# jammm/first_raytracer

Hardware: AMD Instinct MI355X
Metric: Mrays/sec + RMSE vs CPU ref, CornellBox 1080p 512spp, 1/2/4/8 MI355X (higher is better)
Workload: dtype f32

## Files before the change

first_raytracer_amd/__init__.py:

```python
import ctypes
import os

import numpy as np

HERE = os.path.dirname(os.path.abspath(__file__))
LIB_PATH = os.environ.get("FRT_LIB_PATH") or os.path.join(HERE, "libfrt.so")

FRT_WORLD_BVH, FRT_WORLD_LIST = 0, 1
FRT_MAT_LAMBERTIAN, FRT_MAT_DIFFUSE_LIGHT = 0, 1
FRT_PRIM_SPHERE = 1 << 30
ABI_VERSION = 9
FRT_MAT_LAMBERTIAN, FRT_MAT_DIFFUSE_LIGHT, FRT_MAT_MODIFIED_PHONG, FRT_MAT_METAL, FRT_MAT_DIELECTRIC = 0, 1, 2, 3, 4
FRT_MAT_ROUGH_CONDUCTOR = 5
FRT_DIST_GGX, FRT_DIST_BECKMANN = 0, 1
FRT_TEX_CONSTANT, FRT_TEX_CHECKER, FRT_TEX_IMAGE = 0, 1, 2
FRT_IMAGE_SRGB8, FRT_IMAGE_F32 = 0, 1
FRT_FLAG_NO_LDS_SCENE = 1
FRT_FLAG_WAVES5 = 2
FRT_FLAG_WAVES6 = 4
FRT_FLAG_WAVES4 = 8
FRT_FLAG_BVH2 = 16
FRT_FLAG_NO_OCT = 256
FRT_FLAG_FP64 = 512
FRT_FLAG_FP32 = 1024
# ... 96 lines not shown

    @classmethod
    def make(cls, nx, ny, spp, seed=0, max_depth=33, tile_size=32, shard_index=0, shard_count=1,
             samples_per_item=0, flags=0, integrator=0, sample_offset=0):
        return cls(nx=nx, ny=ny, spp=spp, seed=seed, max_depth=max_depth, integrator=integrator, tile_size=tile_size,
                   shard_index=shard_index, shard_count=shard_count, samples_per_item=samples_per_item, flags=flags,
                   mlt_chains=0, mlt_bootstrap=0, sample_offset=sample_offset)

    @classmethod
    def pssmlt(cls, nx, ny, mutations_per_pixel, chains, seed=0, bootstrap=10000, shard_index=0, shard_count=1,
               flags=0):
        return cls(nx=nx, ny=ny, spp=mutations_per_pixel, seed=seed, max_depth=10, integrator=FRT_INTEGRATOR_PSSMLT,
                   tile_size=32, shard_index=shard_index, shard_count=shard_count, samples_per_item=0, flags=flags,
                   mlt_chains=chains, mlt_bootstrap=bootstrap)


class Stats(ctypes.Structure):
    _fields_ = [(n, ctypes.c_uint64) for n in ("camera_rays", "extension_rays", "shadow_rays", "samples",
                                               "pixels", "work_items")] + [
        ("kernel_ms", ctypes.c_double), ("total_ms", ctypes.c_double)] + [
        (n, ctypes.c_uint32) for n in ("scene_in_lds", "waves_cap", "stack_entries", "bvh_depth")] + [
        ("scene_bytes", ctypes.c_uint64), ("fp64", ctypes.c_uint32), ("reserved", ctypes.c_uint32)]

    @property
    def rays(self):
        return self.camera_rays + self.extension_rays + self.shadow_rays

    def as_dict(self):
        d = {n: getattr(self, n) for n, _ in self._fields_}
        d["rays"] = self.rays
        return d


class HostSceneInfo(ctypes.Structure):
    _fields_ = [(n, ctypes.c_int32) for n in ("n_tris", "n_spheres", "n_materials", "n_lights", "n_nodes",
                                              "world_kind", "n_list", "bvh_depth")] + [
        ("load_ms", ctypes.c_double), ("build_ms", ctypes.c_double)]


_lib = None

EXPORTS = ("frt_get_abi_version", "frt_create", "frt_destroy", "frt_last_error", "frt_set_precision", "frt_upload_scene",
           "frt_shard_slot_count", "frt_shard_slots", "frt_render", "frt_render_multi", "frt_render_device", "frt_trace_device",
           "frt_mlt_chain_state",
           "frt_scene_create", "frt_scene_new", "frt_scene_add_obj", "frt_scene_add_sphere", "frt_scene_set_camera",
           "frt_scene_set_env", "frt_scene_add_image", "frt_scene_finish", "frt_scene_build_bvh_gpu",
           "frt_scene_build_bvh_sah", "frt_scene_build_bvh_gpu_algo",
           "frt_scene_view_get", "frt_scene_info", "frt_scene_destroy", "frt_write_tessellated_obj",
           "frt_write_pfm", "frt_film_accumulate", "frt_tonemap_u8", "frt_write_image", "frt_selftest_path_host",
           "frt_selftest_mlt_paths_host",
           "frt_set_env_image", "frt_scene_set_env_image", "frt_scene_env_image", "frt_read_hdr",
           "frt_selftest_path_host_env")


def lib():
    global _lib
    if _lib is not None:
        return _lib
    if not os.path.exists(LIB_PATH):
        raise FrtError(f"{LIB_PATH} is missing: build it with `python -c 'import __graft_entry__ as g; g.build()'`")
    try:
        import torch
    except ImportError:
        pass
    L = ctypes.CDLL(LIB_PATH)
    vp = ctypes.c_void_p
    L.frt_get_abi_version.restype = ctypes.c_int
    if L.frt_get_abi_version() != ABI_VERSION:
        raise FrtError(f"{LIB_PATH}: ABI version {L.frt_get_abi_version()}, binding expects {ABI_VERSION}; rebuild")
    L.frt_create.argtypes = [ctypes.c_int, ctypes.POINTER(vp)]
    L.frt_destroy.argtypes = [vp]
    L.frt_last_error.argtypes = [vp]
    L.frt_last_error.restype = ctypes.c_char_p
    L.frt_set_precision.argtypes = [vp, ctypes.c_int]
    L.frt_upload_scene.argtypes = [vp, ctypes.POINTER(SceneView)]
    L.frt_shard_slot_count.argtypes = [ctypes.POINTER(RenderParams)]
    L.frt_shard_slot_count.restype = ctypes.c_int64
    L.frt_shard_slots.argtypes = [ctypes.POINTER(RenderParams), vp]
    L.frt_render.argtypes = [vp, ctypes.POINTER(RenderParams), vp, ctypes.POINTER(Stats)]
    L.frt_render_device.argtypes = [vp, ctypes.POINTER(RenderParams), vp, vp, ctypes.POINTER(Stats)]
    L.frt_trace_device.argtypes = [vp, vp, ctypes.c_int64, vp, ctypes.c_int, vp, ctypes.POINTER(Stats)]
    L.frt_mlt_chain_state.argtypes = [vp, ctypes.c_uint64, ctypes.c_uint64, vp, vp]
    L.frt_render_multi.argtypes = [ctypes.POINTER(vp), ctypes.c_int, ctypes.POINTER(RenderParams), vp,
                                   ctypes.POINTER(Stats)]
    L.frt_scene_create.argtypes = [ctypes.c_char_p, ctypes.c_char_p, ctypes.c_double, ctypes.POINTER(vp)]
    L.frt_scene_view_get.argtypes = [vp, ctypes.POINTER(SceneView)]
    L.frt_scene_info.argtypes = [vp, ctypes.POINTER(HostSceneInfo)]
    L.frt_scene_destroy.argtypes = [vp]
    L.frt_scene_destroy.restype = None
    dp = ctypes.POINTER(ctypes.c_double)
    L.frt_scene_new.argtypes = [ctypes.POINTER(vp)]
    L.frt_scene_add_obj.argtypes = [vp, ctypes.c_char_p, dp, ctypes.POINTER(Material), ctypes.c_int]
    L.frt_scene_add_sphere.argtypes = [vp, dp, ctypes.c_double, ctypes.POINTER(Material), ctypes.c_int]
    L.frt_scene_set_camera.argtypes = [vp, dp, dp, dp, ctypes.c_double, ctypes.c_double, ctypes.c_double,
                                       ctypes.c_double]
    L.frt_scene_set_env.argtypes = [vp, dp]
    L.frt_scene_add_image.argtypes = [vp, ctypes.POINTER(Image), ctypes.POINTER(ctypes.c_int)]
    L.frt_scene_finish.argtypes = [vp, ctypes.c_int]
    L.frt_scene_build_bvh_gpu.argtypes = [vp, vp, ctypes.POINTER(ctypes.c_double)]
    L.frt_scene_build_bvh_sah.argtypes = [vp]
    L.frt_scene_build_bvh_gpu_algo.argtypes = [vp, vp, ctypes.c_int, ctypes.POINTER(ctypes.c_double)]
    L.frt_write_tessellated_obj.argtypes = [ctypes.c_char_p, ctypes.c_int, ctypes.c_char_p]
    L.frt_write_pfm.argtypes = [ctypes.c_char_p, ctypes.c_int, ctypes.c_int, vp]
    L.frt_film_accumulate.argtypes = [vp, ctypes.c_int64, vp, ctypes.c_int64, ctypes.c_int64]
    L.frt_tonemap_u8.argtypes = [vp, ctypes.c_int, ctypes.c_int, vp]
    L.frt_write_image.argtypes = [ctypes.c_char_p, ctypes.c_int, ctypes.c_int, vp, ctypes.c_int]
    L.frt_selftest_path_host.argtypes = [ctypes.POINTER(SceneView), ctypes.POINTER(RenderParams), vp,
                                         ctypes.c_int, vp, ctypes.POINTER(Stats)]
    L.frt_selftest_mlt_paths_host.argtypes = [ctypes.POINTER(SceneView), ctypes.c_int, ctypes.c_int, ctypes.c_uint32,
                                              ctypes.c_int, vp]
    L.frt_set_env_image.argtypes = [vp, ctypes.POINTER(Image)]
    L.frt_scene_set_env_image.argtypes = [vp, ctypes.c_int]
    L.frt_scene_env_image.argtypes = [vp, ctypes.POINTER(Image)]
    L.frt_read_hdr.argtypes = [ctypes.c_char_p, ctypes.POINTER(ctypes.c_int32), ctypes.POINTER(ctypes.c_int32), vp]
    L.frt_selftest_path_host_env.argtypes = [ctypes.POINTER(SceneView), ctypes.POINTER(RenderParams), vp,
                                             ctypes.c_int, ctypes.POINTER(Image), vp, ctypes.POINTER(Stats)]
    _lib = L
    return L


def _check(rc, what, ctx=None):
    if rc != 0:
        msg = ""
        if ctx is not None:
            msg = lib().frt_last_error(ctx).decode(errors="replace")
        raise FrtError(f"{what} failed: {ERRORS.get(rc, rc)} {msg}")


class HostScene:

    def __init__(self, kind, obj_path, aspect):
        self.ptr = ctypes.c_void_p()
        _check(lib().frt_scene_create(kind.encode(), obj_path.encode(), float(aspect), ctypes.byref(self.ptr)),
               f"frt_scene_create({kind})")
        self.info = HostSceneInfo()
        lib().frt_scene_info(self.ptr, ctypes.byref(self.info))
        self.env = None

    def set_env(self, rgb):
        self.env = tuple(float(x) for x in rgb)

    def set_env_image(self, index):
        _check(lib().frt_scene_set_env_image(self.ptr, -1 if index is None else int(index)), "frt_scene_set_env_image")

    def env_image(self):
        img = Image()
        rc = lib().frt_scene_env_image(self.ptr, ctypes.byref(img))
        if rc < 0:
            _check(rc, "frt_scene_env_image")
# ... 176 lines not shown
    arr = (ctypes.c_void_p * len(contexts))(*[c.ptr for c in contexts])
    st = Stats()
    _check(lib().frt_render_multi(arr, len(contexts), ctypes.byref(params), film.ctypes.data, ctypes.byref(st)),
           "frt_render_multi", contexts[0].ptr)
    return film, st


def shard_slots(params):
    n = lib().frt_shard_slot_count(ctypes.byref(params))
    if n < 0:
        raise FrtError("bad render params")
    out = np.zeros(n, np.int32)
    _check(lib().frt_shard_slots(ctypes.byref(params), out.ctypes.data), "frt_shard_slots")
    return out


def selftest_path_host(scene, params, pixels, env_image=None):
    pixels = np.ascontiguousarray(pixels, dtype=np.int32)
    out = np.zeros((len(pixels), 3), np.float32)
    st = Stats()
    view = scene.view()
    if env_image is None:
        _check(lib().frt_selftest_path_host(ctypes.byref(view), ctypes.byref(params), pixels.ctypes.data, len(pixels),
                                            out.ctypes.data, ctypes.byref(st)), "frt_selftest_path_host")
        return out, st
    a, fmt = image_array({"data": env_image})
    desc = Image(a.shape[1], a.shape[0], fmt, 0, a.ctypes.data)
    _check(lib().frt_selftest_path_host_env(ctypes.byref(view), ctypes.byref(params), pixels.ctypes.data, len(pixels),
                                            ctypes.byref(desc), out.ctypes.data, ctypes.byref(st)),
           "frt_selftest_path_host_env")
    return out, st


def selftest_mlt_paths_host(scene, nx, ny, seed, n):
    out = np.zeros((n, 6), np.float32)
    view = scene.view()
    _check(lib().frt_selftest_mlt_paths_host(ctypes.byref(view), nx, ny, seed, n, out.ctypes.data),
           "frt_selftest_mlt_paths_host")
    return out


def read_hdr(path):
    nx, ny = ctypes.c_int32(0), ctypes.c_int32(0)
    _check(lib().frt_read_hdr(os.fsencode(path), ctypes.byref(nx), ctypes.byref(ny), None), f"frt_read_hdr({path})")
    out = np.zeros((ny.value, nx.value, 3), np.float32)
    _check(lib().frt_read_hdr(os.fsencode(path), ctypes.byref(nx), ctypes.byref(ny), out.ctypes.data),
           f"frt_read_hdr({path})")
    return out


def write_pfm(path, film):
    film = np.ascontiguousarray(film, dtype=np.float32)
    ny, nx = film.shape[0], film.shape[1]
    _check(lib().frt_write_pfm(path.encode(), nx, ny, film.ctypes.data), "frt_write_pfm")


def film_accumulate(acc, acc_spp, film, spp):
    acc = np.ascontiguousarray(acc, dtype=np.float32)
    film = np.ascontiguousarray(film, dtype=np.float32)
    _check(lib().frt_film_accumulate(acc.ctypes.data, int(acc_spp), film.ctypes.data, int(spp), film.size),
           "frt_film_accumulate")
    return acc


def tonemap_u8(film):
    film = np.ascontiguousarray(film, dtype=np.float32)
# ... 28 lines not shown
```

first_raytracer_amd/csrc/frt_flatten.hip:

```cpp
#include "frt_flatten.hpp"

#include <algorithm>
#include <cfloat>
#include <cmath>
#include <cstdlib>
#include <functional>

#include "frt_kernels.hpp"

using namespace frt;

static inline float round_down(double x)
{
    float f = (float)x;
    if ((double)f > x) f = std::nextafter(f, -INFINITY);
    return f;
}
static inline float round_up(double x)
{
    float f = (float)x;
    if ((double)f < x) f = std::nextafter(f, INFINITY);
    return f;
}

static int leaf_size_override()
{
    const char *e = std::getenv("FRT_LEAF_SIZE");
    return e ? std::min(std::max(std::atoi(e), 1), kLeafMax) : 0;
}

static void collapse_leaves(FlatScene &F, int leaf_max)
{
    const int nn = (int)(F.nodes.size() / 4);
    if (leaf_max <= 1 || nn == 0) return;
    auto child = [&](int i, int side) { return f2i(side ? F.nodes[4 * i + 3].y : F.nodes[4 * i + 3].x); };
    std::vector<int> cnt(nn, 0), first(nn, INT32_MAX);
    std::vector<char> sph(nn, 0);
    for (int i = nn - 1; i >= 0; --i)
        for (int side = 0; side < 2; ++side) {
            const int c = child(i, side);
            if (c >= 0) {
// ... 159 lines not shown
    auto srgb = [](double v) { return v <= 0.04045 ? v * (1.0 / 12.92) : std::pow((v + 0.055) * (1.0 / 1.055), 2.4); };
    for (size_t q = 0; q < n; ++q) {
        double c[3];
        for (int ch = 0; ch < 3; ++ch)
            c[ch] = im.format == FRT_IMAGE_F32 ? (double)static_cast<const float *>(im.data)[3 * q + ch]
                                               : srgb(static_cast<const uint8_t *>(im.data)[3 * q + ch] / 255.0);
        out.push_back(make_float4((float)c[0], (float)c[1], (float)c[2], 0.0f));
    }
}
int env_texels_of(const frt_image *img, std::vector<float4> &out, std::string &err)
{
    if (img->nx <= 0 || img->ny <= 0) { err = "environment image: nx and ny must be positive"; return FRT_E_INVALID; }
    if (!img->data) { err = "environment image: null data"; return FRT_E_INVALID; }
    if (img->format != FRT_IMAGE_SRGB8 && img->format != FRT_IMAGE_F32) {
        err = "environment image: format must be FRT_IMAGE_SRGB8 or FRT_IMAGE_F32";
        return FRT_E_INVALID;
    }
    if ((size_t)img->nx * img->ny > (size_t)INT32_MAX) { err = "environment image larger than 2^31 texels"; return FRT_E_UNSUPPORTED; }
    out.clear();
    out.reserve((size_t)img->nx * img->ny);
    append_texels(*img, out);
    for (size_t q = 0; q < out.size(); ++q) {
        const float v[3] = {out[q].x, out[q].y, out[q].z};
        for (int ch = 0; ch < 3; ++ch)
            if (!(v[ch] >= 0.0f && v[ch] <= FLT_MAX)) {
                err = "environment image: texel (" + std::to_string(q % img->nx) + ", " + std::to_string(q / img->nx) +
                      ") is negative or not finite";
                return FRT_E_INVALID;
            }
    }
    return FRT_OK;
}

int flatten_scene(const frt_scene_view *sv, FlatScene &F, std::string &err, bool f64)
{
    auto fail = [&](int code, const std::string &m) { err = m; return code; };
    const int nt = sv->n_tris, ns = sv->n_spheres, nm = sv->n_materials;
    if (nt < 0 || ns < 0 || nm <= 0 || !sv->materials || (nt > 0 && (!sv->tri_v || !sv->tri_material || !sv->tri_inv_area)))
        return fail(FRT_E_INVALID, "scene view: missing triangle arrays or materials");
    if (ns > 0 && (!sv->sphere || !sv->sphere_material)) return fail(FRT_E_INVALID, "scene view: missing sphere arrays");
    for (int i = 0; i < nm; ++i) {
        const int t = sv->materials[i].type;
        if (t != FRT_MAT_LAMBERTIAN && t != FRT_MAT_DIFFUSE_LIGHT && t != FRT_MAT_MODIFIED_PHONG &&
            t != FRT_MAT_METAL && t != FRT_MAT_DIELECTRIC && t != FRT_MAT_ROUGH_CONDUCTOR)
            return fail(FRT_E_UNSUPPORTED, "material type " + std::to_string(t) + " is not supported");
        const int tex = sv->materials[i].texture;
        if (tex != FRT_TEX_CONSTANT && tex != FRT_TEX_CHECKER && tex != FRT_TEX_IMAGE)
            return fail(FRT_E_INVALID, "material texture must be FRT_TEX_CONSTANT, FRT_TEX_CHECKER or FRT_TEX_IMAGE");
        if (tex != FRT_TEX_CONSTANT && (t == FRT_MAT_DIFFUSE_LIGHT || t == FRT_MAT_METAL))
            return fail(FRT_E_UNSUPPORTED, "checker / image textures apply to lambertian / modified_phong / dielectric / "
                                           "rough_conductor colours");
        if (tex == FRT_TEX_IMAGE) {
            const int k = sv->materials[i].image;
            if (k < 0 || k >= sv->n_images || !sv->images)
                return fail(FRT_E_INVALID, "material image index out of range");
            const frt_image &im = sv->images[k];
            if (im.nx <= 0 || im.ny <= 0 || !im.data || (im.format != FRT_IMAGE_SRGB8 && im.format != FRT_IMAGE_F32))
                return fail(FRT_E_INVALID, "scene view: bad image");
        }
        if (t == FRT_MAT_ROUGH_CONDUCTOR &&
            (!(sv->materials[i].alpha > 0.0) || (sv->materials[i].distribution != FRT_DIST_GGX &&
                                                  sv->materials[i].distribution != FRT_DIST_BECKMANN)))
            return fail(FRT_E_INVALID, "rough_conductor needs alpha > 0 and a GGX / Beckmann distribution");
    }
    auto valid_ref = [&](int ref) {
        if (ref < 0) return false;
        if (ref & FRT_PRIM_SPHERE) return (ref & ~FRT_PRIM_SPHERE) < ns;
// ... 184 lines not shown
        const size_t n = (size_t)im.nx * im.ny;
        if (F.texels.size() + n > (size_t)INT32_MAX) return fail(FRT_E_UNSUPPORTED, "images larger than 2^31 texels");
        image_off[k] = (int)F.texels.size();
        append_texels(im, F.texels);
    }
    F.mats.assign(kMatStride * (size_t)nm, make_float4(0.0f, 0.0f, 0.0f, 0.0f));
    for (int i = 0; i < nm; ++i) {
        const frt_material &m = sv->materials[i];
        float4 *d = &F.mats[kMatStride * i];
        auto f4 = [](const double *v, float w) { return make_float4((float)v[0], (float)v[1], (float)v[2], w); };
        d[0] = f4(m.type == FRT_MAT_ROUGH_CONDUCTOR ? m.eta : m.albedo, i2f(m.type));
        if (m.type == FRT_MAT_DIFFUSE_LIGHT) d[1] = f4(m.emit, 0.0f);
        else d[1] = f4(m.specular, (float)(m.type == FRT_MAT_MODIFIED_PHONG ? m.exponent
                                           : m.type == FRT_MAT_DIELECTRIC ? m.ior : m.alpha));
        d[2] = f4(m.k, i2f(m.distribution));
        d[3] = f4(m.tex_odd, i2f(m.texture));
        d[4] = make_float4((float)m.tex_scale[0], (float)m.tex_scale[1], 0.0f, 0.0f);
        if (m.texture == FRT_TEX_IMAGE)
            d[4] = make_float4(i2f(sv->images[m.image].nx), i2f(sv->images[m.image].ny), i2f(image_off[m.image]), 0.0f);
    }
    if (sv->n_lights < 0 || (sv->n_lights > 0 && !sv->lights)) return fail(FRT_E_INVALID, "scene view: bad lights");
    F.lights.resize(sv->n_lights);
    for (int i = 0; i < sv->n_lights; ++i) {
        if (!valid_ref(sv->lights[i])) return fail(FRT_E_INVALID, "scene view: bad light");
        F.lights[i] = dev_ref(sv->lights[i]);
    }
    F.list.resize(sv->world_kind == FRT_WORLD_LIST ? sv->n_list : 0);
    for (size_t i = 0; i < F.list.size(); ++i) F.list[i] = dev_ref(sv->list[i]);

    const size_t oct_bytes = sizeof(float4) * (oct_lds_node_slots((int)(F.nodes.size() / 4)) + F.tris.size() +
                                               F.tshade.size() + F.mats.size());
    if (sv->world_kind == FRT_WORLD_BVH && F.depth < kLdsMaxDepth && oct_bytes <= kLdsOctBytes)
        F.nodes_oct.resize(8 * F.nodes.size());
    for (int o = 0; o < 8 && !F.nodes_oct.empty(); ++o)
        for (size_t i = 0; i < F.nodes.size() / 4; ++i) {
            const float4 *n = &F.nodes[4 * i];
            const float b0[6] = {n[0].x, n[0].y, n[0].z, n[0].w, n[1].x, n[1].y};
            const float b1[6] = {n[1].z, n[1].w, n[2].x, n[2].y, n[2].z, n[2].w};
            float q[12];
            for (int a = 0; a < 3; ++a) {
                const bool neg = (o >> a) & 1;
                q[a] = neg ? b0[3 + a] : b0[a];
                q[3 + a] = neg ? b0[a] : b0[3 + a];
                q[6 + a] = neg ? b1[3 + a] : b1[a];
                q[9 + a] = neg ? b1[a] : b1[3 + a];
            }
            float4 *d = &F.nodes_oct[(size_t)o * F.nodes.size() + 4 * i];
            d[0] = make_float4(q[0], q[1], q[2], q[3]);
            d[1] = make_float4(q[4], q[5], q[6], q[7]);
            d[2] = make_float4(q[8], q[9], q[10], q[11]);
            d[3] = n[3];
        }
    S.root = (sv->world_kind == FRT_WORLD_BVH) ? ((sv->root >= 0) ? 0 : ~dev_ref(~sv->root)) : 0;
    F.has4 = sv->world_kind == FRT_WORLD_BVH && build_bvh4(F, S.root);
    if (!F.has4) F.nodes4.clear();
    S.root4 = F.has4 ? F.root4 : S.root;
    S.n_lights = sv->n_lights;
    S.n_list = (int)F.list.size();
    S.n_nodes = (int)(F.nodes.size() / 4);
    S.n_tris = nt;
    S.n_mats = nm;
    S.n_nodes4 = (int)(F.nodes4.size() / kNode4Parts);
    S.node_es = 4; S.node_ps = 1;
    S.node4_es = kNode4Parts; S.node4_ps = 1;
    S.tri_es = 3; S.tri_ps = 1;
    S.sh_es = 2; S.sh_ps = 1;
    S.world_kind = sv->world_kind;
    auto f3d = [](const double *x) { return mk3((float)x[0], (float)x[1], (float)x[2]); };
    S.cam_o = f3d(sv->cam_origin); S.cam_llc = f3d(sv->cam_lower_left);
    S.cam_h = f3d(sv->cam_horizontal); S.cam_v = f3d(sv->cam_vertical);
    S.cam_u = f3d(sv->cam_u); S.cam_vv = f3d(sv->cam_v);
    S.lens_r = (float)sv->cam_lens_radius;
    S.cam_w = f3d(sv->cam_w);
    S.cam_half_height = (float)sv->cam_half_height;
    S.env = f3d(sv->env_color);
    auto d3d = [](const double *x) { return d3{x[0], x[1], x[2]}; };
    S.cam64_o = d3d(sv->cam_origin); S.cam64_llc = d3d(sv->cam_lower_left);
    S.cam64_h = d3d(sv->cam_horizontal); S.cam64_v = d3d(sv->cam_vertical);
    S.cam64_u = d3d(sv->cam_u); S.cam64_vv = d3d(sv->cam_v);
    S.lens_r64 = sv->cam_lens_radius;
    return FRT_OK;
}

DevScene host_scene(const FlatScene &F)
{
    DevScene S = F.meta;
    S.nodes = F.nodes.data(); S.nodes4 = F.nodes4.data(); S.nodes_oct = F.nodes_oct.data();
    S.tris = F.tris.data(); S.tshade = F.tshade.data(); S.tnorm = F.tnorm.data();
    S.tuv = F.tuv.data(); S.texels = F.texels.data();
    S.spheres = F.spheres.data(); S.sphere_mat = F.smat.data(); S.mats = F.mats.data();
    S.lights = F.lights.data(); S.list = F.list.data(); S.tri_view = F.tri_view.data();
    S.tris64 = F.tris64.data(); S.tshade64 = F.tshade64.data(); S.tnorm64 = F.tnorm64.data();
    S.spheres64 = F.spheres64.data();
    return S;
}
```

first_raytracer_amd/csrc/frt_flatten.hpp:

```cpp
#pragma once
#include <string>
#include <vector>

#include "frt.h"
#include "frt_device.hpp"
#include "frt_path.hpp"

using frt::DevScene;

#pragma GCC visibility push(hidden)
struct FlatScene {
    std::vector<float4> nodes, tris, tshade, tnorm, spheres, mats, tuv;
    std::vector<float4> texels;
    std::vector<uint4> nodes4;
    std::vector<float4> nodes_oct;
    std::vector<double4> tris64, tshade64, tnorm64, spheres64;
    bool has4 = false;
    int root4 = 0, depth4 = 0;
    std::vector<int> smat, lights, list;
    std::vector<int> tri_view;
    DevScene meta{};
    int depth = 0;
};

int flatten_scene(const frt_scene_view *sv, FlatScene &F, std::string &err, bool f64);
int env_texels_of(const frt_image *img, std::vector<float4> &out, std::string &err);
frt::DevScene host_scene(const FlatScene &F);
#pragma GCC visibility pop
```

first_raytracer_amd/csrc/frt_selftest.hip:

```cpp
#include <algorithm>
#include <cstring>
#include <string>
#include <vector>

#include "frt_ctx.hpp"
#include "frt_flatten.hpp"
#include "host/envdist.hpp"

using namespace frt;

constexpr int kSelftestStack = 8;

template <typename R, int MATS = kMatsAll>
static void selftest_pixels(const DevScene &S, const FlatScene &F, const frt_render_params *p, const int32_t *pixels,
                            int npix, bool wide, std::vector<int> &stack, float *out_rgb, uint64_t cnt[3])
{
    uint32_t n_ext = 0, n_sh = 0;
    for (int i = 0; i < npix; ++i) {
        const int pix = pixels[i];
        const int px = pix % p->nx, py = pix / p->nx;
        V3<R> acc = zero3<R>();
        for (int smp = 0; smp < p->spp; ++smp) {
            PathState<R> P;
            path_begin<MATS>(P, S, px, py, p->nx, p->ny, p->seed, (uint32_t)pix, (uint32_t)(smp + p->sample_offset));
// ... 102 lines not shown
    }
    return FRT_OK;
}


extern "C" int frt_selftest_mlt_paths_host(const frt_scene_view *sv, int nx, int ny, uint32_t seed, int n,
                                           float *out6)
{
    if (!sv || !out6 || n < 0 || nx <= 0 || ny <= 0) return FRT_E_INVALID;
    FlatScene F;
    std::string err;
    const int rc = flatten_scene(sv, F, err, false);
    if (rc != FRT_OK) return rc;
    const DevScene S = host_scene(F);
    std::vector<int> stack(std::max(F.depth + 1, 1));
    for (int i = 0; i < n; ++i) {
        PrndSource src{nullptr, 0, 0, rng_key(seed ^ kMltBootSalt, (uint32_t)i, 0u), 0u, true, 0.0f, 0.0f};
        MltPath M;
        mlt_begin(M, S, src, nx, ny);
        uint32_t ne = 0, ns = 0;
        for (;;) {
            if (mlt_beyond(M)) { M.P.L = M.P.L + M.P.beta * env_of<float>(S); break; }
            const Hit<float> h = (S.world_kind == FRT_WORLD_LIST)
                              ? trace<FRT_WORLD_LIST, 1>(S, M.P.ro, M.P.rd, M.P.rtmax, M.P.shadow, stack.data())
                              : trace<FRT_WORLD_BVH, 1>(S, M.P.ro, M.P.rd, M.P.rtmax, M.P.shadow, stack.data());
            if (mlt_shade(M, S, h, src, ne, ns)) break;
        }
        const f3 L = M.P.L;
        float *o = &out6[6 * (size_t)i];
        o[0] = M.x; o[1] = M.y; o[2] = L.x; o[3] = L.y; o[4] = L.z; o[5] = fmaxf(fmaxf(L.x, L.y), L.z);
    }
    return FRT_OK;
}
```

include/frt.h:

```cpp
#ifndef FRT_H
#define FRT_H

#include <stdint.h>

#ifdef __cplusplus
extern "C" {
#endif

#define FRT_ABI_VERSION 9

enum {
    FRT_OK = 0,
    FRT_E_INVALID = -1,
    FRT_E_HIP = -2,
    FRT_E_NO_SCENE = -3,
    FRT_E_UNSUPPORTED = -4,
    FRT_E_IO = -5,
    FRT_E_NO_DEVICE = -6
};

enum { FRT_WORLD_BVH = 0, FRT_WORLD_LIST = 1 };
enum { FRT_MAT_LAMBERTIAN = 0,
       FRT_MAT_DIFFUSE_LIGHT = 1,
       FRT_MAT_MODIFIED_PHONG = 2,
// ... 158 lines not shown
int frt_scene_add_obj(frt_host_scene *s, const char *obj_path, const double *to_world16, const frt_material *bsdf,
                      int use_geometry_normals);
int frt_scene_add_sphere(frt_host_scene *s, const double *center, double radius, const frt_material *m, int where);
int frt_scene_set_camera(frt_host_scene *s, const double *lookfrom, const double *lookat, const double *vup,
                         double vfov, double aspect, double aperture, double focus_dist);
int frt_scene_set_env(frt_host_scene *s, const double *rgb);
int frt_scene_add_image(frt_host_scene *s, const frt_image *img, int *index);
int frt_scene_set_env_image(frt_host_scene *s, int index);
int frt_scene_env_image(const frt_host_scene *s, frt_image *out);
int frt_scene_finish(frt_host_scene *s, int world_kind);
enum { FRT_GPU_BVH_PLOC = 0, FRT_GPU_BVH_LBVH = 1, FRT_GPU_BVH_SAH = 2 };
int frt_scene_build_bvh_gpu(frt_host_scene *s, frt_ctx *ctx, double *device_ms);
int frt_scene_build_bvh_gpu_algo(frt_host_scene *s, frt_ctx *ctx, int algo, double *device_ms);
int frt_scene_build_bvh_sah(frt_host_scene *s);
int frt_scene_info(const frt_host_scene *s, frt_host_scene_info *info);
void frt_scene_destroy(frt_host_scene *s);

int frt_write_tessellated_obj(const char *src_obj, int k, const char *dst_obj);

int frt_read_hdr(const char *path, int32_t *nx, int32_t *ny, float *rgb);

int frt_write_pfm(const char *path, int nx, int ny, const float *rgb);

int frt_film_accumulate(float *acc, int64_t acc_spp, const float *pass, int64_t pass_spp, int64_t n);
int frt_tonemap_u8(const float *rgb, int nx, int ny, uint8_t *out_u8);
enum { FRT_IMAGE_PNG = 0, FRT_IMAGE_BMP = 1, FRT_IMAGE_JPG = 2 };
int frt_write_image(const char *path, int nx, int ny, const uint8_t *rgb_u8, int format);

int frt_selftest_path_host(const frt_scene_view *scene, const frt_render_params *p, const int32_t *pixels,
                           int npix, float *out_rgb, frt_stats *st);
int frt_selftest_path_host_env(const frt_scene_view *scene, const frt_render_params *p, const int32_t *pixels,
                               int npix, const frt_image *env, float *out_rgb, frt_stats *st);
int frt_selftest_mlt_paths_host(const frt_scene_view *scene, int nx, int ny, uint32_t seed, int n, float *out6);

#ifdef __cplusplus
}
#endif
#endif
```

Baseline: 33560.

## Refine BVH topology on host with ray-sampled subtree reinsertion cost search

Adds a host-side BVH refinement pass that samples path-traced rays over a small frame and measures per-ray node visits and primitive tests. It then greedily reinserts subtrees to minimize a weighted cost, keeping the new tree only if it also lowers cost on a separate validation ray set. The octant node copies and the BVH4 tree are rebuilt from the refined tree, and refinement is on by default for LDS-resident scenes. The aim is fewer traversal steps per ray, paid for with extra host work at scene upload and a tree tuned to sampled rays from one camera.

```diff
diff --git a/first_raytracer_amd/__init__.py b/first_raytracer_amd/__init__.py
--- a/first_raytracer_amd/__init__.py
+++ b/first_raytracer_amd/__init__.py
@@ -152,6 +152,15 @@
         return d
 
 
+class TreeCost(ctypes.Structure):
+    _fields_ = [("v", ctypes.c_double), ("t", ctypes.c_double), ("j", ctypes.c_double), ("w", ctypes.c_double),
+                ("depth", ctypes.c_int32), ("n_nodes", ctypes.c_int32), ("n_rays", ctypes.c_int32),
+                ("applies", ctypes.c_int32)]
+
+    def as_dict(self):
+        return {k: getattr(self, k) for k, _ in self._fields_}
+
+
 class HostSceneInfo(ctypes.Structure):
     _fields_ = [(n, ctypes.c_int32) for n in ("n_tris", "n_spheres", "n_materials", "n_lights", "n_nodes",
                                               "world_kind", "n_list", "bvh_depth")] + [
@@ -171,6 +180,7 @@
            "frt_selftest_mlt_paths_host",
            "frt_set_env_image", "frt_scene_set_env_image", "frt_scene_env_image", "frt_read_hdr",
            "frt_selftest_path_host_env")
+EXPORTS_X = ("frtx_selftest_tree_refine", "frtx_selftest_trace_host")
 
 
 def lib():
@@ -235,6 +245,8 @@
     L.frt_read_hdr.argtypes = [ctypes.c_char_p, ctypes.POINTER(ctypes.c_int32), ctypes.POINTER(ctypes.c_int32), vp]
     L.frt_selftest_path_host_env.argtypes = [ctypes.POINTER(SceneView), ctypes.POINTER(RenderParams), vp,
                                              ctypes.c_int, ctypes.POINTER(Image), vp, ctypes.POINTER(Stats)]
+    L.frtx_selftest_tree_refine.argtypes = [ctypes.POINTER(SceneView), ctypes.POINTER(TreeCost), vp, vp, ctypes.c_int32]
+    L.frtx_selftest_trace_host.argtypes = [ctypes.POINTER(SceneView), vp, ctypes.c_int64, vp]
     _lib = L
     return L
 
@@ -477,6 +489,25 @@
     return out, st
 
 
+def selftest_tree_refine(scene):
+    view = scene.view()
+    cap = max(1, view.n_tris + view.n_spheres)
+    nodes = [np.zeros((cap, 16), np.float32) for _ in range(2)]
+    out = (TreeCost * 2)()
+    _check(lib().frtx_selftest_tree_refine(ctypes.byref(view), out, nodes[0].ctypes.data, nodes[1].ctypes.data, cap),
+           "frtx_selftest_tree_refine")
+    return tuple((out[k].as_dict(), nodes[k][:out[k].n_nodes].copy()) for k in range(2))
+
+
+def selftest_trace_host(scene, rays):
+    rays = np.ascontiguousarray(rays, dtype=np.float32).reshape(-1, 8)
+    hits = np.zeros((len(rays), 4), np.float32)
+    view = scene.view()
+    _check(lib().frtx_selftest_trace_host(ctypes.byref(view), rays.ctypes.data, len(rays), hits.ctypes.data),
+           "frtx_selftest_trace_host")
+    return hits
+
+
 def selftest_mlt_paths_host(scene, nx, ny, seed, n):
     out = np.zeros((n, 6), np.float32)
     view = scene.view()
diff --git a/first_raytracer_amd/csrc/frt_flatten.hip b/first_raytracer_amd/csrc/frt_flatten.hip
--- a/first_raytracer_amd/csrc/frt_flatten.hip
+++ b/first_raytracer_amd/csrc/frt_flatten.hip
@@ -7,6 +7,7 @@
 #include <functional>
 
 #include "frt_kernels.hpp"
+#include "host/tree_refine.hpp"
 
 using namespace frt;
 
@@ -232,7 +233,202 @@
     return FRT_OK;
 }
 
-int flatten_scene(const frt_scene_view *sv, FlatScene &F, std::string &err, bool f64)
+static void fill_octants(FlatScene &F)
+{
+    for (int o = 0; o < 8 && !F.nodes_oct.empty(); ++o)
+        for (size_t i = 0; i < F.nodes.size() / 4; ++i) {
+            const float4 *n = &F.nodes[4 * i];
+            const float b0[6] = {n[0].x, n[0].y, n[0].z, n[0].w, n[1].x, n[1].y};
+            const float b1[6] = {n[1].z, n[1].w, n[2].x, n[2].y, n[2].z, n[2].w};
+            float q[12];
+            for (int a = 0; a < 3; ++a) {
+                const bool neg = (o >> a) & 1;
+                q[a] = neg ? b0[3 + a] : b0[a];
+                q[3 + a] = neg ? b0[a] : b0[3 + a];
+                q[6 + a] = neg ? b1[3 + a] : b1[a];
+                q[9 + a] = neg ? b1[a] : b1[3 + a];
+            }
+            float4 *d = &F.nodes_oct[(size_t)o * F.nodes.size() + 4 * i];
+            d[0] = make_float4(q[0], q[1], q[2], q[3]);
+            d[1] = make_float4(q[4], q[5], q[6], q[7]);
+            d[2] = make_float4(q[8], q[9], q[10], q[11]);
+            d[3] = n[3];
+        }
+}
+
+constexpr double kRefineW = 1.8;
+constexpr int kRefineFitFrame = 24, kRefineValFrame = 40;
+constexpr uint32_t kRefineFitSeed = 0x7ee5eed1u, kRefineValSeed = 0x7ee5eed2u;
+constexpr int kRefineMaxDepth = 33;
+constexpr int kRefineMaxEvals = 700;
+
+static bool tree_refine_knob()
+{
+    const char *e = std::getenv("FRT_TREE_REFINE");
+    return !(e && std::atoi(e) == 0);
+}
+
+static bool tree_in_lds(const FlatScene &F)
+{
+    if (F.meta.world_kind != FRT_WORLD_BVH || F.meta.root < 0 || F.depth >= kLdsMaxDepth) return false;
+    const size_t bytes = sizeof(float4) * (F.nodes.size() + F.tris.size() + F.tshade.size() + F.mats.size());
+    return bytes <= kLdsSceneBytes || !F.nodes_oct.empty();
+}
+
+struct RefineLeaf { float box[6]; int ref; };
+
+static void topology_of(const std::vector<float4> &nodes, frt_refine::Topology &t, std::vector<RefineLeaf> &leaves)
+{
+    const int nn = (int)(nodes.size() / 4);
+    leaves.clear();
+    t.child.assign(2 * (size_t)nn, 0);
+    t.n_leaves = nn + 1;
+    t.root = t.n_leaves;
+    for (int i = 0; i < nn; ++i) {
+        const float4 *n = &nodes[4 * i];
+        const float b[2][6] = {{n[0].x, n[0].y, n[0].z, n[0].w, n[1].x, n[1].y}, {n[1].z, n[1].w, n[2].x, n[2].y, n[2].z, n[2].w}};
+        for (int side = 0; side < 2; ++side) {
+            const int c = f2i(side ? n[3].y : n[3].x);
+            if (c >= 0) { t.child[2 * i + side] = t.n_leaves + c; continue; }
+            RefineLeaf l;
+            for (int k = 0; k < 6; ++k) l.box[k] = b[side][k];
+            l.ref = c;
+            t.child[2 * i + side] = (int)leaves.size();
+            leaves.push_back(l);
+        }
+    }
+}
+
+static void sample_rays(const FlatScene &F, const std::vector<RefineLeaf> &leaves, int frame, uint32_t seed,
+                        frt_refine::RaySet &R)
+{
+    const DevScene S = host_scene(F);
+    struct Ray { f3 o, d; float tmax; bool shadow; };
+    std::vector<Ray> rays;
+    std::vector<int> stack(std::max(F.depth + 1, 1));
+    for (int pix = 0; pix < frame * frame; ++pix) {
+        PathState<float> P;
+        path_begin<kMatsAll>(P, S, pix % frame, pix / frame, frame, frame, seed, (uint32_t)pix, 0u);
+        for (;;) {
+            rays.push_back(Ray{P.ro, P.rd, P.rtmax, P.shadow});
+            const Hit<float> h = trace<FRT_WORLD_BVH, 1>(S, P.ro, P.rd, P.rtmax, P.shadow, stack.data());
+            uint32_t n_ext = 0, n_sh = 0;
+            if (path_shade<kMatsAll>(P, S, h, kRefineMaxDepth, n_ext, n_sh)) break;
+        }
+    }
+    const int n = (int)rays.size(), nl = (int)leaves.size();
+    R = frt_refine::RaySet{};
+    R.n = n;
+    R.n_leaves = nl;
+    R.prim_first.assign(nl + 1, 0);
+    for (int l = 0; l < nl; ++l) {
+        const int lref = ~leaves[l].ref;
+        const bool sph = (lref & FRT_PRIM_SPHERE) != 0;
+        const int first = sph ? lref : (lref & kLeafIndexMask), count = sph ? 1 : (lref >> kLeafCountShift) + 1;
+        for (int k = 0; k < count; ++k) R.prim_ref.push_back(first + k);
+        R.prim_first[l + 1] = (int)R.prim_ref.size();
+    }
+    R.n_prims = (int)R.prim_ref.size();
+    R.tmin.resize(n); R.tmax.resize(n); R.anyhit.resize(n); R.live.resize(n);
+    R.slab.resize((size_t)nl * n * 6);
+    R.prim_t.resize((size_t)n * R.n_prims);
+    int stride = (int)(0.618 * n) | 1;
+    auto gcd = [](int a, int b) { while (b) { const int c = a % b; a = b; b = c; } return a; };
+    while (n > 1 && gcd(stride, n) != 1) stride += 2;
+    for (int i = 0; i < n; ++i) {
+        const Ray &q = rays[(int)(((int64_t)i * stride) % std::max(n, 1))];
+        Trav<float> T;
+        R.live[i] = trav_begin(T, S, S.root, q.o, q.d, q.tmax) ? 1 : 0;
+        R.tmin[i] = T.tmin;
+        R.tmax[i] = q.tmax;
+        R.anyhit[i] = q.shadow ? 1 : 0;
+        const float inv[3] = {T.sr.invd.x, T.sr.invd.y, T.sr.invd.z}, oi[3] = {T.sr.oinv.x, T.sr.oinv.y, T.sr.oinv.z};
+        for (int l = 0; l < nl; ++l) {
+            float *s = &R.slab[((size_t)i * nl + l) * 6];
+            for (int a = 0; a < 3; ++a) {
+                const bool neg = inv[a] < 0.0f;
+                s[a] = vfma(leaves[l].box[neg ? 3 + a : a], inv[a], oi[a]);
+                s[3 + a] = -vfma(leaves[l].box[neg ? a : 3 + a], inv[a], oi[a]);
+            }
+        }
+        for (int k = 0; k < R.n_prims; ++k) {
+            float u, v;
+            R.prim_t[(size_t)i * R.n_prims + k] = prim_t(S, R.prim_ref[k], q.o, q.d, T.tmin, q.tmax, u, v);
+        }
+    }
+}
+
+static void write_topology(FlatScene &F, const frt_refine::Topology &t, const std::vector<RefineLeaf> &leaves)
+{
+    const int L = t.n_leaves, nn = L - 1;
+    std::vector<float> box(6 * (size_t)(L + nn));
+    std::function<void(int)> bound = [&](int s) {
+        float *b = &box[6 * (size_t)s];
+        if (s < L) { for (int k = 0; k < 6; ++k) b[k] = leaves[s].box[k]; return; }
+        const int c0 = t.child[2 * (s - L)], c1 = t.child[2 * (s - L) + 1];
+        bound(c0);
+        bound(c1);
+        for (int k = 0; k < 3; ++k) {
+            b[k] = std::min(box[6 * (size_t)c0 + k], box[6 * (size_t)c1 + k]);
+            b[3 + k] = std::max(box[6 * (size_t)c0 + 3 + k], box[6 * (size_t)c1 + 3 + k]);
+        }
+    };
+    bound(t.root);
+    std::vector<float4> out(4 * (size_t)nn);
+    int next = 0;
+    std::function<int(int)> emit = [&](int s) {
+        if (s < L) return leaves[s].ref;
+        const int me = next++;
+        const int c[2] = {t.child[2 * (s - L)], t.child[2 * (s - L) + 1]};
+        const float *a = &box[6 * (size_t)c[0]], *b = &box[6 * (size_t)c[1]];
+        out[4 * me + 0] = make_float4(a[0], a[1], a[2], a[3]);
+        out[4 * me + 1] = make_float4(a[4], a[5], b[0], b[1]);
+        out[4 * me + 2] = make_float4(b[2], b[3], b[4], b[5]);
+        const int r0 = emit(c[0]), r1 = emit(c[1]);
+        out[4 * me + 3] = make_float4(i2f(r0), i2f(r1), 0.0f, 0.0f);
+        return me;
+    };
+    emit(t.root);
+    F.nodes.swap(out);
+}
+
+bool tree_cost_host(const FlatScene &F, TreeCost &out)
+{
+    out = TreeCost{};
+    out.w = kRefineW;
+    if (!tree_in_lds(F) || F.nodes.empty()) return false;
+    frt_refine::Topology t;
+    std::vector<RefineLeaf> leaves;
+    topology_of(F.nodes, t, leaves);
+    frt_refine::RaySet val;
+    sample_rays(F, leaves, kRefineValFrame, kRefineValSeed, val);
+    const frt_refine::Cost c = frt_refine::tree_cost(t, val);
+    out.V = c.V; out.T = c.T; out.J = frt_refine::cost_j(c, kRefineW);
+    out.depth = t.depth();
+    out.n_rays = val.n;
+    return true;
+}
+
+static bool refine_tree(FlatScene &F)
+{
+    if (!tree_in_lds(F) || F.nodes.size() / 4 < 3) return false;
+    frt_refine::Topology t;
+    std::vector<RefineLeaf> leaves;
+    topology_of(F.nodes, t, leaves);
+    const frt_refine::Topology input = t;
+    frt_refine::RaySet fit;
+    sample_rays(F, leaves, kRefineFitFrame, kRefineFitSeed, fit);
+    if (frt_refine::refine(t, fit, kRefineW, input.depth(), kRefineMaxEvals) == 0) return false;
+    frt_refine::RaySet val;
+    sample_rays(F, leaves, kRefineValFrame, kRefineValSeed, val);
+    const double j0 = frt_refine::cost_j(frt_refine::tree_cost(input, val), kRefineW);
+    const double j1 = frt_refine::cost_j(frt_refine::tree_cost(t, val), kRefineW);
+    if (!(j1 < j0)) return false;
+    write_topology(F, t, leaves);
+    return true;
+}
+
+int flatten_scene(const frt_scene_view *sv, FlatScene &F, std::string &err, bool f64, int refine)
 {
     auto fail = [&](int code, const std::string &m) { err = m; return code; };
     const int nt = sv->n_tris, ns = sv->n_spheres, nm = sv->n_materials;
@@ -483,29 +679,15 @@
                                                F.tshade.size() + F.mats.size());
     if (sv->world_kind == FRT_WORLD_BVH && F.depth < kLdsMaxDepth && oct_bytes <= kLdsOctBytes)
         F.nodes_oct.resize(8 * F.nodes.size());
-    for (int o = 0; o < 8 && !F.nodes_oct.empty(); ++o)
-        for (size_t i = 0; i < F.nodes.size() / 4; ++i) {
-            const float4 *n = &F.nodes[4 * i];
-            const float b0[6] = {n[0].x, n[0].y, n[0].z, n[0].w, n[1].x, n[1].y};
-            const float b1[6] = {n[1].z, n[1].w, n[2].x, n[2].y, n[2].z, n[2].w};
-            float q[12];
-            for (int a = 0; a < 3; ++a) {
-                const bool neg = (o >> a) & 1;
-                q[a] = neg ? b0[3 + a] : b0[a];
-                q[3 + a] = neg ? b0[a] : b0[3 + a];
-                q[6 + a] = neg ? b1[3 + a] : b1[a];
-                q[9 + a] = neg ? b1[a] : b1[3 + a];
-            }
-            float4 *d = &F.nodes_oct[(size_t)o * F.nodes.size() + 4 * i];
-            d[0] = make_float4(q[0], q[1], q[2], q[3]);
-            d[1] = make_float4(q[4], q[5], q[6], q[7]);
-            d[2] = make_float4(q[8], q[9], q[10], q[11]);
-            d[3] = n[3];
-        }
     S.root = (sv->world_kind == FRT_WORLD_BVH) ? ((sv->root >= 0) ? 0 : ~dev_ref(~sv->root)) : 0;
-    F.has4 = sv->world_kind == FRT_WORLD_BVH && build_bvh4(F, S.root);
-    if (!F.has4) F.nodes4.clear();
-    S.root4 = F.has4 ? F.root4 : S.root;
+    auto derive_trees = [&]() {
+        fill_octants(F);
+        F.has4 = sv->world_kind == FRT_WORLD_BVH && build_bvh4(F, S.root);
+        if (!F.has4) F.nodes4.clear();
+        S.root4 = F.has4 ? F.root4 : S.root;
+        S.n_nodes4 = (int)(F.nodes4.size() / kNode4Parts);
+    };
+    derive_trees();
     S.n_lights = sv->n_lights;
     S.n_list = (int)F.list.size();
     S.n_nodes = (int)(F.nodes.size() / 4);
@@ -530,6 +712,7 @@
     S.cam64_h = d3d(sv->cam_horizontal); S.cam64_v = d3d(sv->cam_vertical);
     S.cam64_u = d3d(sv->cam_u); S.cam64_vv = d3d(sv->cam_v);
     S.lens_r64 = sv->cam_lens_radius;
+    if ((refine < 0 ? tree_refine_knob() : refine != 0) && refine_tree(F)) derive_trees();
     return FRT_OK;
 }
 
diff --git a/first_raytracer_amd/csrc/frt_flatten.hpp b/first_raytracer_amd/csrc/frt_flatten.hpp
--- a/first_raytracer_amd/csrc/frt_flatten.hpp
+++ b/first_raytracer_amd/csrc/frt_flatten.hpp
@@ -23,7 +23,9 @@
     int depth = 0;
 };
 
-int flatten_scene(const frt_scene_view *sv, FlatScene &F, std::string &err, bool f64);
+int flatten_scene(const frt_scene_view *sv, FlatScene &F, std::string &err, bool f64, int refine = -1);
+struct TreeCost { double V = 0.0, T = 0.0, J = 0.0, w = 0.0; int depth = 0, n_rays = 0; };
+bool tree_cost_host(const FlatScene &F, TreeCost &out);
 int env_texels_of(const frt_image *img, std::vector<float4> &out, std::string &err);
 frt::DevScene host_scene(const FlatScene &F);
 #pragma GCC visibility pop
diff --git a/first_raytracer_amd/csrc/frt_selftest.hip b/first_raytracer_amd/csrc/frt_selftest.hip
--- a/first_raytracer_amd/csrc/frt_selftest.hip
+++ b/first_raytracer_amd/csrc/frt_selftest.hip
@@ -158,3 +158,49 @@
     }
     return FRT_OK;
 }
+
+extern "C" int frtx_selftest_tree_refine(const frt_scene_view *sv, frt_tree_cost out[2], float *nodes_off,
+                                        float *nodes_on, int32_t max_nodes)
+{
+    if (!sv || !out) return FRT_E_INVALID;
+    float *dst[2] = {nodes_off, nodes_on};
+    for (int on = 0; on < 2; ++on) {
+        FlatScene F;
+        std::string err;
+        const int rc = flatten_scene(sv, F, err, false, on);
+        if (rc != FRT_OK) return rc;
+        TreeCost c;
+        const bool applies = tree_cost_host(F, c);
+        const int nn = (int)(F.nodes.size() / 4);
+        out[on] = frt_tree_cost{c.V, c.T, c.J, c.w, c.depth, nn, c.n_rays, applies ? 1 : 0};
+        if (dst[on]) {
+            if (nn > max_nodes) return FRT_E_INVALID;
+            memcpy(dst[on], F.nodes.data(), F.nodes.size() * sizeof(float4));
+        }
+    }
+    return FRT_OK;
+}
+
+extern "C" int frtx_selftest_trace_host(const frt_scene_view *sv, const float *rays, int64_t n, float *hits)
+{
+    if (!sv || n < 0 || (n > 0 && (!rays || !hits))) return FRT_E_INVALID;
+    FlatScene F;
+    std::string err;
+    const int rc = flatten_scene(sv, F, err, false);
+    if (rc != FRT_OK) return rc;
+    const DevScene S = host_scene(F);
+    std::vector<int> stack(std::max(F.depth + 1, 1));
+    for (int64_t i = 0; i < n; ++i) {
+        const float *q = rays + 8 * i;
+        const f3 o = mk3(q[0], q[1], q[2]), d = mk3(q[4], q[5], q[6]);
+        const bool anyhit = (f2i(q[7]) & 1) != 0;
+        const Hit<float> h = S.world_kind == FRT_WORLD_LIST ? trace<FRT_WORLD_LIST, 1>(S, o, d, q[3], anyhit, stack.data())
+                                                            : trace<FRT_WORLD_BVH, 1>(S, o, d, q[3], anyhit, stack.data());
+        const int ref = (h.prim < 0 || (h.prim & FRT_PRIM_SPHERE)) ? h.prim : F.tri_view[h.prim];
+        float *r = hits + 4 * i;
+        r[0] = h.t; r[1] = h.u; r[2] = h.v;
+        const float refbits = i2f(ref);
+        memcpy(&r[3], &refbits, sizeof(float));
+    }
+    return FRT_OK;
+}
diff --git a/first_raytracer_amd/csrc/host/tree_refine.cpp b/first_raytracer_amd/csrc/host/tree_refine.cpp
--- /dev/null
+++ b/first_raytracer_amd/csrc/host/tree_refine.cpp
@@ -0,0 +1,235 @@
+#include "tree_refine.hpp"
+
+#include <algorithm>
+#include <cstddef>
+#include <cstring>
+
+#include "frt.h"
+
+namespace frt_refine {
+namespace {
+
+constexpr int kMaxLevels = 64;
+constexpr int kChunks = 16;
+constexpr double kSlack = 0.002;
+
+struct Tables {
+    int n_slots = 0;
+    std::vector<float> tab;
+};
+
+inline void unite(const float *a, const float *b, float *out)
+{
+    for (int k = 0; k < 6; ++k) out[k] = std::min(a[k], b[k]);
+}
+
+void count_rays(const Topology &t, const RaySet &R, const Tables &tb, const int *dirty, int n_dirty, const int *local_of,
+                int r0, int r1, uint64_t &V, uint64_t &T)
+{
+    const int L = t.n_leaves;
+    const int *child = t.child.data();
+    float loc[2 * kMaxLevels][6];
+    for (int r = r0; r < r1; ++r) {
+        if (!R.live[r]) continue;
+        const float *base = &tb.tab[(size_t)r * tb.n_slots * 6];
+        auto rec = [&](int s) { return n_dirty > 0 && local_of[s] >= 0 ? loc[local_of[s]] : base + 6 * s; };
+        for (int k = 0; k < n_dirty; ++k) {
+            const int j = dirty[k] - L;
+            unite(rec(child[2 * j]), rec(child[2 * j + 1]), loc[k]);
+        }
+        const float tmin = R.tmin[r];
+        const bool any = R.anyhit[r] != 0;
+        const float *pt = &R.prim_t[(size_t)r * R.n_prims];
+        float tb_ = R.tmax[r];
+        int hp = -1, sp = 0, node = t.root;
+        int stk[kMaxLevels];
+        for (;;) {
+            while (node >= L) {
+                ++V;
+                const int c0 = child[2 * (node - L)], c1 = child[2 * (node - L) + 1];
+                const float *a = rec(c0), *b = rec(c1);
+                const float t0 = std::max(std::max(a[0], a[1]), std::max(a[2], tmin));
+                const float f0 = std::min(std::min(-a[3], -a[4]), std::min(-a[5], tb_));
+                const float t1 = std::max(std::max(b[0], b[1]), std::max(b[2], tmin));
+                const float f1 = std::min(std::min(-b[3], -b[4]), std::min(-b[5], tb_));
+                const bool h0 = t0 <= f0, h1 = t1 <= f1;
+                if (h0 && h1) {
+                    const bool first0 = t0 <= t1;
+                    stk[sp++] = first0 ? c1 : c0;
+                    node = first0 ? c0 : c1;
+                } else if (h0) {
+                    node = c0;
+                } else if (h1) {
+                    node = c1;
+                } else {
+                    node = sp > 0 ? stk[--sp] : -1;
+                }
+            }
+            if (node < 0) break;
+            bool done = false;
+            for (int k = R.prim_first[node]; k < R.prim_first[node + 1]; ++k) {
+                ++T;
+                const float th = pt[k];
+                const int ref = R.prim_ref[k];
+                const bool sph = (ref & FRT_PRIM_SPHERE) != 0;
+                if (th > 0.0f && th <= tb_ && (th < tb_ || (sph ? hp >= 0 : ref < hp))) {
+                    tb_ = th;
+                    hp = ref;
+                    if (any) { done = true; break; }
+                }
+            }
+            if (done || sp == 0) break;
+            node = stk[--sp];
+        }
+    }
+}
+
+void build_tables(const Topology &t, const RaySet &R, Tables &tb)
+{
+    const int L = t.n_leaves, nI = std::max(L - 1, 0);
+    tb.n_slots = L + nI;
+    tb.tab.resize((size_t)R.n * tb.n_slots * 6);
+    std::vector<int> order, st{t.root};
+    while (!st.empty()) {
+        const int s = st.back();
+        st.pop_back();
+        if (s < L) continue;
+        order.push_back(s);
+        st.push_back(t.child[2 * (s - L)]);
+        st.push_back(t.child[2 * (s - L) + 1]);
+    }
+    for (int r = 0; r < R.n; ++r) {
+        float *base = &tb.tab[(size_t)r * tb.n_slots * 6];
+        memcpy(base, &R.slab[(size_t)r * L * 6], sizeof(float) * 6 * L);
+        for (size_t k = order.size(); k-- > 0;) {
+            const int s = order[k], j = s - L;
+            unite(base + 6 * t.child[2 * j], base + 6 * t.child[2 * j + 1], base + 6 * s);
+        }
+    }
+}
+
+}
+
+int Topology::depth() const
+{
+    int d = 0, sp = 0;
+    int st[2 * kMaxLevels][2];
+    st[sp][0] = root; st[sp++][1] = 1;
+    while (sp > 0) {
+        const int s = st[--sp][0], lvl = st[sp][1];
+        if (s < n_leaves) continue;
+        d = std::max(d, lvl);
+        if (lvl >= kMaxLevels) return lvl;
+        st[sp][0] = child[2 * (s - n_leaves)]; st[sp++][1] = lvl + 1;
+        st[sp][0] = child[2 * (s - n_leaves) + 1]; st[sp++][1] = lvl + 1;
+    }
+    return d;
+}
+
+Cost tree_cost(const Topology &t, const RaySet &R)
+{
+    Tables tb;
+    build_tables(t, R, tb);
+    uint64_t V = 0, T = 0;
+    count_rays(t, R, tb, nullptr, 0, nullptr, 0, R.n, V, T);
+    Cost c;
+    if (R.n > 0) { c.V = (double)V / R.n; c.T = (double)T / R.n; }
+    return c;
+}
+
+int refine(Topology &t, const RaySet &R, double w, int max_depth, int max_evals)
+{
+    const int L = t.n_leaves, nI = L - 1, nS = L + nI;
+    if (nI < 2 || R.n <= 0 || max_depth >= kMaxLevels) return 0;
+    Tables tb;
+    std::vector<int> parent(nS, -1), local_of(nS, -1);
+    int bound[kChunks + 1];
+    for (int c = 0; c <= kChunks; ++c) bound[c] = (int)((int64_t)R.n * c / kChunks);
+    double prefix[kChunks + 1] = {0.0};
+    auto keep_tree = [&]() {
+        std::fill(parent.begin(), parent.end(), -1);
+        for (int j = 0; j < nI; ++j) { parent[t.child[2 * j]] = L + j; parent[t.child[2 * j + 1]] = L + j; }
+        build_tables(t, R, tb);
+        uint64_t V = 0, T = 0;
+        for (int c = 0; c < kChunks; ++c) {
+            count_rays(t, R, tb, nullptr, 0, nullptr, bound[c], bound[c + 1], V, T);
+            prefix[c + 1] = (double)V + w * (double)T;
+        }
+    };
+    keep_tree();
+    auto in_subtree = [&](int x, int s) {
+        for (; x >= 0; x = parent[x]) if (x == s) return true;
+        return false;
+    };
+    auto side_of = [&](int par, int c) { return 2 * (par - L) + (t.child[2 * (par - L)] == c ? 0 : 1); };
+    auto move = [&](int s, int x) {
+        const int p = parent[s];
+        const int q = t.child[side_of(p, s) ^ 1];
+        const int g = parent[p];
+        if (g < 0) t.root = q;
+        else t.child[side_of(g, p)] = q;
+        parent[q] = g;
+        const int xp = parent[x];
+        if (xp < 0) t.root = p;
+        else t.child[side_of(xp, x)] = p;
+        parent[p] = xp;
+        t.child[2 * (p - L)] = x;
+        t.child[2 * (p - L) + 1] = s;
+        parent[x] = p;
+        parent[s] = p;
+        return g;
+    };
+    int evals = 0, kept = 0;
+    bool improved = true;
+    while (improved && evals < max_evals) {
+        improved = false;
+        for (int s = 0; s < nS && evals < max_evals; ++s) {
+            if (parent[s] < 0) continue;
+            int best_x = -1;
+            double best_j = prefix[kChunks];
+            const Topology keep = t;
+            const std::vector<int> keep_parent = parent;
+            const int p = parent[s], q = t.child[side_of(p, s) ^ 1];
+            for (int x = 0; x < nS && evals < max_evals; ++x) {
+                if (x == p || x == q || in_subtree(x, s)) continue;
+                const int g = move(s, x);
+                if (t.depth() <= max_depth) {
+                    ++evals;
+                    std::pair<int, int> dl[2 * kMaxLevels];
+                    int nd = 0;
+                    for (int start : {p, g})
+                        for (int y = start; y >= 0; y = parent[y]) {
+                            int lvl = 0;
+                            for (int z = y; z >= 0; z = parent[z]) ++lvl;
+                            dl[nd++] = {-lvl, y};
+                        }
+                    std::sort(dl, dl + nd);
+                    nd = (int)(std::unique(dl, dl + nd) - dl);
+                    int dirty[2 * kMaxLevels];
+                    for (int k = 0; k < nd; ++k) { dirty[k] = dl[k].second; local_of[dirty[k]] = k; }
+                    uint64_t V = 0, T = 0;
+                    const double slack = kSlack * prefix[kChunks];
+                    double j = 0.0;
+                    bool ok = true;
+                    for (int c = 0; c < kChunks && ok; ++c) {
+                        count_rays(t, R, tb, dirty, nd, local_of.data(), bound[c], bound[c + 1], V, T);
+                        j = (double)V + w * (double)T;
+                        ok = j <= prefix[c + 1] + slack;
+                    }
+                    for (int k = 0; k < nd; ++k) local_of[dirty[k]] = -1;
+                    if (ok && j < best_j) { best_j = j; best_x = x; }
+                }
+                t = keep;
+                parent = keep_parent;
+            }
+            if (best_x < 0) continue;
+            move(s, best_x);
+            keep_tree();
+            ++kept;
+            improved = true;
+        }
+    }
+    return kept;
+}
+
+}
diff --git a/first_raytracer_amd/csrc/host/tree_refine.hpp b/first_raytracer_amd/csrc/host/tree_refine.hpp
--- /dev/null
+++ b/first_raytracer_amd/csrc/host/tree_refine.hpp
@@ -0,0 +1,30 @@
+#pragma once
+#include <cstdint>
+#include <vector>
+
+namespace frt_refine {
+
+struct RaySet {
+    int n = 0, n_leaves = 0, n_prims = 0;
+    std::vector<float> tmin, tmax;
+    std::vector<uint8_t> anyhit, live;
+    std::vector<float> slab;
+    std::vector<int> prim_first;
+    std::vector<int> prim_ref;
+    std::vector<float> prim_t;
+};
+
+struct Topology {
+    int n_leaves = 0, root = 0;
+    std::vector<int> child;
+    int depth() const;
+};
+
+struct Cost { double V = 0.0, T = 0.0; };
+inline double cost_j(const Cost &c, double w) { return c.V + w * c.T; }
+
+Cost tree_cost(const Topology &t, const RaySet &rays);
+
+int refine(Topology &t, const RaySet &fit, double w, int max_depth, int max_evals);
+
+}
diff --git a/include/frt.h b/include/frt.h
--- a/include/frt.h
+++ b/include/frt.h
@@ -214,6 +214,13 @@
 int frt_selftest_path_host_env(const frt_scene_view *scene, const frt_render_params *p, const int32_t *pixels,
                                int npix, const frt_image *env, float *out_rgb, frt_stats *st);
 int frt_selftest_mlt_paths_host(const frt_scene_view *scene, int nx, int ny, uint32_t seed, int n, float *out6);
+typedef struct frt_tree_cost {
+    double v, t, j, w;
+    int32_t depth, n_nodes, n_rays, applies;
+} frt_tree_cost;
+int frtx_selftest_tree_refine(const frt_scene_view *scene, frt_tree_cost out[2], float *nodes_off, float *nodes_on,
+                             int32_t max_nodes);
+int frtx_selftest_trace_host(const frt_scene_view *scene, const float *rays, int64_t n, float *hits);
 
 #ifdef __cplusplus
 }
```

Result: faster. 35400, median of 6 (+5.5%).
